# Samirez/Visual_odometry

Measured on AMD Instinct MI355X. Metric: frame-pairs/sec (1280x720, 2000 ORB feats), higher is better.
Workload: dtype u8+f32+f64; 1 GPU; seeded synthetic 1280x720 drone flight (256 distinct rendered views, closed loop), 2000 ORB features/frame, 8 levels = BASELINE config 2; chunk of 257 consecutive frames -> 256 pairs (k, k+1) per GPU per step, each frame detected once; detector=orb, distinct_rendered_frames=256, pair_stride=1, contexts_per_gpu=3, keypoint_order=cv2, poly_solver=fast, matcher=crosscheck, matcher_kernel=mfma_fp4, ransac=5-point, conf 0.99, 1 px, seed 2^64-1, <=1000 iters, parallelism=single GPU, pairs_ok_last_step=256

## Files before the change

### visual_odometry_amd/csrc/orb_kernels.hip

```cpp
#include "vo_internal.h"
#include <type_traits>
#include <float.h>
#include <stdlib.h>

__constant__ int8_t c_pattern[256 * 4] = {
#include "orb_pattern.inc"
};
__constant__ int c_umax[16] = {15, 15, 15, 15, 14, 14, 14, 13, 13, 12, 11, 10, 9, 8, 6, 3};
__constant__ int c_gauss7[7] = {18, 34, 49, 55, 49, 34, 18};


typedef short vo_s16x2 __attribute__((ext_vector_type(2)));
typedef unsigned short vo_u16x2 __attribute__((ext_vector_type(2)));
__device__ __forceinline__ uint32_t pk_sub16(uint32_t a, uint32_t b)
{
    return __builtin_bit_cast(uint32_t, __builtin_bit_cast(vo_s16x2, a) - __builtin_bit_cast(vo_s16x2, b));
}
__device__ __forceinline__ uint32_t pk_add16(uint32_t a, uint32_t b)
{
    return __builtin_bit_cast(uint32_t, __builtin_bit_cast(vo_s16x2, a) + __builtin_bit_cast(vo_s16x2, b));
}
__device__ __forceinline__ uint32_t pk_min16(uint32_t a, uint32_t b)
{
    return __builtin_bit_cast(uint32_t, __builtin_elementwise_min(__builtin_bit_cast(vo_s16x2, a), __builtin_bit_cast(vo_s16x2, b)));
// ... 1310 lines not shown
        uint32_t h0[4], h1[4];
        uint32_t a0 = src[0][0], a1 = src[0][1], a2 = src[0][2], b0 = src[1][0], b1 = src[1][1], b2 = src[1][2];
        if (EDGE) { bd_fix(a0, a1, a2, e); bd_fix(b0, b1, b2, e); }
        bd_hpass(a0, a1, a2, h0); bd_hpass(b0, b1, b2, h1);
#pragma unroll
        for (int c = 0; c < 4; c++) q[c] = h0[c] | (h1[c] << 16);
    };
#pragma unroll
    for (int u = 0; u < BD_AHEAD; u++) fetch(u, W[u]);
#pragma unroll
    for (int k = 0; k < 3; k++) {
        hstep(W[k % BD_AHEAD], Q[k % 4]);
        fetch(k + BD_AHEAD, W[k % BD_AHEAD]);
    }
    uint32_t orow = (uint32_t)(y0 * lv.stride);
    for (int m0 = 0; m0 < nsteps; m0 += 4) {
#pragma unroll
        for (int j = 0; j < 4; j++) {
            const int m = m0 + j;
            if (m >= nsteps) break;
            constexpr int K0 = 3;
            const int ki = (K0 + j) % 4, wi = (K0 + j) % BD_AHEAD;
            hstep(W[wi], Q[ki]);
            fetch(K0 + m + BD_AHEAD, W[wi]);
            const uint32_t r0 = bd_vrow<false>(Q[(ki + 1) % 4], Q[(ki + 2) % 4], Q[(ki + 3) % 4], Q[ki]);
            const uint32_t r1 = bd_vrow<true>(Q[(ki + 1) % 4], Q[(ki + 2) % 4], Q[(ki + 3) % 4], Q[ki]);
            __builtin_amdgcn_raw_buffer_store_b32(r0, drs, col_ok ? (uint32_t)x + orow : 0xfffffff0u, 0, 0);
            __builtin_amdgcn_raw_buffer_store_b32(r1, drs, col_ok && 2 * m + 1 < nout ? (uint32_t)x + orow + (uint32_t)lv.stride : 0xfffffff0u, 0, 0);
            orow += 2u * (uint32_t)lv.stride;
        }
    }
}

__global__ __launch_bounds__(256) void k_blur_direct(const uint8_t* pyr, uint8_t* blur, PyrGeom g, int total)
{
    const int f = blockIdx.y, lane = threadIdx.x & 63, wave = __builtin_amdgcn_readfirstlane(threadIdx.x >> 6);
    const int wt = xcd_tile(blockIdx.x, gridDim.x) * 4 + wave;
    if (wt >= total) return;
    int l = 0, first = 0;
    for (;;) {
        const int nt = ((g.lv[l].stride + 255) / 256) * ((g.lv[l].h + BD_R - 1) / BD_R);
        if (wt < first + nt || l + 1 == g.nlevels) break;
        first += nt; l++;
    }
    const LevelGeom lv = g.lv[l];
    const int ntx = (lv.stride + 255) / 256, tile = wt - first;
    const int x0 = (tile % ntx) * 256, y0 = (tile / ntx) * BD_R;
    const int x = x0 + 4 * lane;
    const uint8_t* img = pyr + (size_t)f * g.frame_bytes + lv.off;
    const int xb = min(max(x - 4, 0), lv.stride - 12);
    BdEdge e;
    e.left = x0 == 0; e.right = x0 + 256 + 8 > lv.w;
    e.shl = x == 0; e.shr = x - 4 > lv.stride - 12 && x < lv.stride;
    {
        const int d = lv.w - x;
        e.s1 = d == 1 ? 0x01020304u : d == 2 ? 0x03040504u : d == 3 ? 0x05060504u : 0x07060504u;
        e.s2 = d == 2 ? 0x0c0c0c02u : d == 3 ? 0x0c0c0304u : 0x0c040506u;
        e.s3 = d == 5 ? 0x01020304u : d == 6 ? 0x03040504u : 0x07060504u;
        e.use_t = d >= 2 && d <= 4;
    }
    const __amdgpu_buffer_rsrc_t drs = __builtin_amdgcn_make_buffer_rsrc(blur + (size_t)f * g.frame_bytes + lv.off, 0, lv.stride * lv.h, 0x00020000);
    const bool col_ok = x < lv.stride;
    const int nout = min(BD_R, lv.h - y0);
    const int nsteps = (nout + 1) / 2;
    const bool inside = y0 >= 3 && y0 - 3 + 2 * (nsteps + 3 + BD_AHEAD) <= lv.h, edge = e.left || e.right;
    if (inside && !edge) bd_strip<true, false>(img, lv, drs, x, xb, y0, nout, nsteps, col_ok, e);
    else if (inside) bd_strip<true, true>(img, lv, drs, x, xb, y0, nout, nsteps, col_ok, e);
    else if (!edge) bd_strip<false, false>(img, lv, drs, x, xb, y0, nout, nsteps, col_ok, e);
    else bd_strip<false, true>(img, lv, drs, x, xb, y0, nout, nsteps, col_ok, e);
}

void launch_blur(hipStream_t s, const uint8_t* pyr, uint8_t* blur, const PyrGeom& g, int F)
{
    bool direct = true;
    int total = 0;
    for (int l = 0; l < g.nlevels; l++) {
        direct = direct && g.lv[l].w >= 16 && g.lv[l].h >= 8;
        total += ((g.lv[l].stride + 255) / 256) * ((g.lv[l].h + BD_R - 1) / BD_R);
    }
    if (direct) { hipLaunchKernelGGL(k_blur_direct, dim3((total + 3) / 4, F), dim3(256), 0, s, pyr, blur, g, total); return; }
    hipLaunchKernelGGL(k_blur, dim3(g.btiles_total, F), dim3(256), 0, s, pyr, blur, g);
}

__device__ __forceinline__ uint32_t brief_expand4(uint32_t nib)
{
    const uint32_t m = (nib * 0x00204081u) & 0x01010101u;
    return 0x81818181u ^ (m * 0xfeu);
}

__device__ __forceinline__ uint32_t brief_expand8_fp4(uint32_t b)
{
    uint32_t w = (b | (b << 12)) & 0x000F000Fu;
    w = (w | (w << 6)) & 0x03030303u;
    w = (w | (w << 3)) & 0x11111111u;
    return 0xAAAAAAAAu ^ (w << 3);
}

__global__ __launch_bounds__(256) void k_brief_trig(PyrGeom g, FrameFeat ff)
{
    const int f = blockIdx.y, k = blockIdx.x * 256 + threadIdx.x;
    if (k >= min(ff.kp_count[f], g.kp_cap)) return;
    const size_t ki = (size_t)f * g.kp_cap + k;
    const float angle = ff.kp_angle[ki] * (float)(3.1415926535897932384626433832795 / 180.f);
    ff.kp_xy[ki * 2] = (float)cos((double)angle);
    ff.kp_xy[ki * 2 + 1] = (float)sin((double)angle);
}

#define BR_R 18
#define BR_ROWS (2 * BR_R + 1)
#ifndef BR_KPW
#define BR_KPW 2
#endif
__global__ __launch_bounds__(256) void k_brief(const uint8_t* blur, PyrGeom g, FrameFeat ff, uint8_t* desc_x, int cap_x, int blocks_per_frame, int fp4)
{
    __shared__ __attribute__((aligned(16))) uint8_t s_win[4][BR_KPW][BR_ROWS * 64];
    const int bid = xcd_tile(blockIdx.x, gridDim.x);
    const int f = bid / blocks_per_frame, lane = threadIdx.x & 63, wave = threadIdx.x >> 6;
    const int k0 = ((bid % blocks_per_frame) * 4 + wave) * BR_KPW;
    const int cnt = min(ff.kp_count[f], g.kp_cap);
    if (k0 >= cnt) return;
    float ca[BR_KPW], cb[BR_KPW], kxs[BR_KPW], kys[BR_KPW], sfs[BR_KPW];
    int coff[BR_KPW];
    uint4 wv[BR_KPW][3];
#pragma unroll
    for (int q = 0; q < BR_KPW; q++) {
        const size_t ki = (size_t)f * g.kp_cap + min(k0 + q, cnt - 1);
        const uint32_t pos = __builtin_amdgcn_readfirstlane(ff.kp_pos[ki]);
        const int level = __builtin_amdgcn_readfirstlane(ff.kp_level[ki]);
        const float sf = g.lv[level].scale;
        const int stride = g.lv[level].stride, lh = g.lv[level].h;
        const float kx = (float)(pos & 0xffff) * sf, ky = (float)(pos >> 16) * sf;
        const float inv = 1.f / sf;
        const int cx = __float2int_rn(kx * inv), cy = __float2int_rn(ky * inv);
        ca[q] = ff.kp_xy[ki * 2]; cb[q] = ff.kp_xy[ki * 2 + 1];
        kxs[q] = kx; kys[q] = ky; sfs[q] = sf;
        const uint8_t* img = blur + (size_t)f * g.frame_bytes + g.lv[level].off;
        const int xs = (cx - BR_R) & ~15;
        const int nchunk = (cx - BR_R - xs) + 2 * BR_R + 1 > 48 ? 4 : 3;
        coff[q] = BR_R * 64 + (cx - xs);
#pragma unroll
        for (int it = 0; it < 3; it++) {
            const int idx = min(it * 64 + lane, BR_ROWS * 4 - 1);
            const int r = idx >> 2, c = idx & 3;
            const int gy = min(max(cy - BR_R + r, 0), lh - 1), gx = min(max(xs + (c < nchunk ? 16 * c : 0), 0), stride - 16);
            wv[q][it] = *(const uint4*)(img + (size_t)gy * stride + gx);
        }
    }
#pragma unroll
    for (int q = 0; q < BR_KPW; q++)
#pragma unroll
        for (int it = 0; it < 3; it++) {
            const int idx = it * 64 + lane;
            if (idx < BR_ROWS * 4) *(uint4*)(s_win[wave][q] + idx * 16) = wv[q][it];
        }
#pragma unroll
    for (int q = 0; q < BR_KPW; q++) {
        const int k = k0 + q;
        if (k >= cnt) break;
        const size_t ki = (size_t)f * g.kp_cap + k;
        const uint8_t* center = s_win[wave][q] + coff[q];
        const float a = ca[q], b = cb[q];
        uint64_t words[4];
#pragma unroll
        for (int w = 0; w < 4; w++) {
            const int8_t* pt = c_pattern + (w * 64 + lane) * 4;
            const float px0 = (float)pt[0], py0 = (float)pt[1], px1 = (float)pt[2], py1 = (float)pt[3];
            const float xa = px0 * a - py0 * b, ya = px0 * b + py0 * a;
            const float xb = px1 * a - py1 * b, yb = px1 * b + py1 * a;
            const int t0 = center[__float2int_rn(ya) * 64 + __float2int_rn(xa)];
            const int t1 = center[__float2int_rn(yb) * 64 + __float2int_rn(xb)];
            words[w] = __ballot(t0 < t1);
        }
        if (lane < 4) {
            uint64_t wv8 = lane == 0 ? words[0] : lane == 1 ? words[1] : lane == 2 ? words[2] : words[3];
            *(uint64_t*)(ff.desc + ki * 32 + lane * 8) = wv8;
        }
        if (fp4 < 0) {
        } else if (fp4) {
            if (lane < 8) {
                const uint64_t wv8 = lane < 2 ? words[0] : lane < 4 ? words[1] : lane < 6 ? words[2] : words[3];
                const uint32_t bits = (uint32_t)(wv8 >> (32 * (lane & 1)));
                const uint4 o = make_uint4(brief_expand8_fp4(bits & 255u), brief_expand8_fp4((bits >> 8) & 255u), brief_expand8_fp4((bits >> 16) & 255u), brief_expand8_fp4(bits >> 24));
                *(uint4*)(desc_x + ((size_t)f * cap_x * 16 + (size_t)(k & ~15) * 8 + (size_t)lane * 16 + (k & 15)) * 16) = o;
            }
        } else if (lane < 16) {
            const uint64_t wv8 = lane < 4 ? words[0] : lane < 8 ? words[1] : lane < 12 ? words[2] : words[3];
            const uint32_t bits = (uint32_t)(wv8 >> (16 * (lane & 3))) & 0xffffu;
            const uint4 o = make_uint4(brief_expand4(bits & 15u), brief_expand4((bits >> 4) & 15u), brief_expand4((bits >> 8) & 15u), brief_expand4(bits >> 12));
            *(uint4*)(desc_x + (((size_t)f * cap_x + (k & ~15)) * 16 + (size_t)lane * 16 + (k & 15)) * 16) = o;
        }
        if (lane == 0) {
            ff.kp_xy[ki * 2] = kxs[q]; ff.kp_xy[ki * 2 + 1] = kys[q];
            ff.kp_size[ki] = 31 * sfs[q];
        }
    }
}

void launch_brief(hipStream_t s, const uint8_t* blur, const PyrGeom& g, FrameFeat ff, int F, uint8_t* desc_x, int cap_x, int fp4)
{
    hipLaunchKernelGGL(k_brief_trig, dim3((g.kp_cap + 255) / 256, F), dim3(256), 0, s, g, ff);
    const int bpf = (g.kp_cap + 4 * BR_KPW - 1) / (4 * BR_KPW);
    hipLaunchKernelGGL(k_brief, dim3(bpf * F), dim3(256), 0, s, blur, g, ff, desc_x, cap_x, bpf, -1);
    launch_desc_expand(s, ff.desc, ff.kp_count, g.kp_cap, cap_x, desc_x, F, fp4);
}
```

### visual_odometry_amd/csrc/vo_api.hip

```cpp
#include "vo_internal.h"
#include <float.h>
#include <math.h>
#include <stdio.h>
#include <stdlib.h>
#include <string.h>
#include <vector>
#include <type_traits>
#include <algorithm>

#define MAX_EVENTS 384

struct DevList {
    struct Entry { void* p; bool pinned; };
    std::vector<Entry> ptrs;
    DevList() = default;
    DevList(const DevList&) = delete;
    DevList& operator=(DevList&& o) noexcept { if (this != &o) { release(); ptrs.swap(o.ptrs); } return *this; }
    ~DevList() { release(); }
    template <typename T> hipError_t alloc(T** p, size_t n) { return keep(hipMalloc((void**)p, (n ? n : 1) * sizeof(T)), (void**)p, false); }
    template <typename T> hipError_t alloc_pinned(T** p, size_t n)
    {
        return keep(hipHostMalloc((void**)p, (n ? n : 1) * sizeof(T), hipHostMallocDefault), (void**)p, true);
    }
    void release()
// ... 407 lines not shown
}

extern "C" int vo_set_poly_solver(vo_ctx* ctx, int kind)
{
    if (!ctx) return VO_ERR_INVALID;
    if (kind != 0 && kind != 1) FAIL(VO_ERR_INVALID, "poly solver must be 0 (noise-floor exit) or 1 (OpenCV's fixed 300 sweeps)");
    ctx->dk_early = kind == 0;
    return VO_OK;
}

extern "C" int vo_set_pnp_refine(vo_ctx* ctx, int kind)
{
    if (!ctx) return VO_ERR_INVALID;
    if (kind != 0 && kind != 1) FAIL(VO_ERR_INVALID, "pnp refine must be 1 (cv2's solvePnP(ITERATIVE) on the inliers) or 0 (fast minimiser from the RANSAC model)");
    ctx->pnp_refine = kind;
    return VO_OK;
}

extern "C" const char* vo_last_error(const vo_ctx* ctx) { return ctx ? ctx->err : "ctx is NULL"; }

extern "C" int vo_batch_configure(vo_ctx* ctx, int h, int w, const vo_orb_params* params, int max_frames, int max_pairs)
{
    if (!ctx) return VO_ERR_INVALID;
    int rc = check_params(ctx, params);
    if (rc) return rc;
    if (h < 1 || w < 1 || max_frames < 1 || max_pairs < 1) FAIL(VO_ERR_INVALID, "bad sizes");
    HIPCHK(hipSetDevice(ctx->device));
    if (ctx->configured && ctx->h == h && ctx->w == w && memcmp(&ctx->params, params, sizeof(*params)) == 0 &&
        ctx->max_frames >= max_frames && ctx->max_pairs >= max_pairs && ctx->pb_cap == ctx->g.kp_cap) {
        ctx->detector = 0;
        clear_last_run(ctx);
        return VO_OK;
    }
    HIPCHK(hipStreamSynchronize(ctx->stream));
    free_config(ctx);
    PyrGeom g;
    rc = make_geometry(ctx, h, w, params, &g);
    if (rc) return rc;
    ctx->g = g; ctx->h = h; ctx->w = w; ctx->params = *params;
    ctx->max_frames = max_frames; ctx->max_pairs = max_pairs;

    size_t tab_ints = 0, tab_u16 = 0;
    for (int l = 1; l < g.nlevels; l++) { tab_ints += g.lv[l].w + g.lv[l].h; tab_u16 += g.lv[l].w + g.lv[l].h; }
    std::vector<int> hofs(tab_ints + 1);
    std::vector<uint16_t> hc(tab_u16 + 1);
    const size_t int_bytes = (tab_ints + 1) * sizeof(int);
    DevList& m = ctx->orb_mem;
    uint8_t* tab_mem = nullptr;
    HIPCHK(m.alloc(&tab_mem, int_bytes + (tab_u16 + 1) * sizeof(uint16_t) + 64));
    int* d_ofs = (int*)tab_mem;
    uint16_t* d_c = (uint16_t*)(tab_mem + int_bytes);
    size_t oi = 0;
    for (int l = 1; l < g.nlevels; l++) {
        ResizeTab& t = ctx->tabs[l];
        const LevelGeom &s = g.lv[l - 1], &d = g.lv[l];
        build_lin_tab(s.w, d.w, &hofs[oi], &hc[oi], &t.min_x, &t.max_x);
        t.xofs = d_ofs + oi; t.xc1 = d_c + oi; oi += d.w;
        build_lin_tab(s.h, d.h, &hofs[oi], &hc[oi], &t.min_y, &t.max_y);
        t.yofs = d_ofs + oi; t.yc1 = d_c + oi; oi += d.h;
        {
            const int* xo = &hofs[oi - d.h - d.w]; const int* yo = &hofs[oi - d.h];
            bool ok = true;
            for (int x = 0; x + 3 < d.w && ok; x++) ok = xo[x + 3] - xo[x] <= 4;
            for (int y = 0; y + 1 < d.h && ok; y++) ok = yo[y + 1] > yo[y];
            for (int y0 = 0; y0 < d.h && ok; y0 += RS2_WH) { const int yl = (y0 + RS2_WH < d.h ? y0 + RS2_WH : d.h) - 1; ok = yo[yl] + 2 - yo[y0] <= (RS2_WH * 127 + 99) / 100 + 3; }
            t.direct = ok ? 1 : 0;
        }
    }
    HIPCHK(hipMemcpy(d_ofs, hofs.data(), int_bytes, hipMemcpyHostToDevice));
    HIPCHK(hipMemcpy(d_c, hc.data(), (tab_u16 + 1) * sizeof(uint16_t), hipMemcpyHostToDevice));

    const size_t F = (size_t)max_frames, fb = (size_t)g.frame_bytes;
    HIPCHK(m.alloc(&ctx->pyr, F * fb + 256));
    HIPCHK(m.alloc(&ctx->blur, F * fb));
    HIPCHK(m.alloc(&ctx->score, F * fb));
    HIPCHK(hipMemset(ctx->pyr, 0, F * fb));
    FrameFeat& ff = ctx->ff;
    HIPCHK(m.alloc(&ff.cand_pos, F * g.cand_total)); HIPCHK(m.alloc(&ff.cand_resp, F * g.cand_total));
    HIPCHK(m.alloc(&ff.cand_count, F * VO_MAX_LEVELS));
    HIPCHK(m.alloc(&ff.kp_pos, F * g.kp_cap)); HIPCHK(m.alloc(&ff.kp_level, F * g.kp_cap));
    HIPCHK(m.alloc(&ff.kp_resp, F * g.kp_cap)); HIPCHK(m.alloc(&ff.kp_angle, F * g.kp_cap));
    HIPCHK(m.alloc(&ff.kp_xy, F * g.kp_cap * 2)); HIPCHK(m.alloc(&ff.kp_size, F * g.kp_cap));
    HIPCHK(m.alloc(&ff.desc, F * g.kp_cap * 32));
    HIPCHK(m.alloc(&ctx->desc_x, F * (size_t)desc_x_rows(g.kp_cap) * 256));
    HIPCHK(hipMemset(ctx->desc_x, 0xFF, F * (size_t)desc_x_rows(g.kp_cap) * 256));
    HIPCHK(m.alloc(&ff.kp_count, F)); HIPCHK(m.alloc(&ff.flags, F));
    HIPCHK(m.alloc(&ff.hist, F * VO_MAX_LEVELS * 256));
    HIPCHK(m.alloc(&ff.tile_list, F * (size_t)g.ftiles_total * FAST_LISTCAP));
    HIPCHK(m.alloc(&ff.tile_count, F * (size_t)g.ftiles_total));
    HIPCHK(m.alloc(&ctx->sel_thr, F * VO_MAX_LEVELS));
    HIPCHK(m.alloc(&ctx->har_kept, F * VO_MAX_LEVELS));
    HIPCHK(m.alloc(&ctx->har_thr, F * VO_MAX_LEVELS));
    HIPCHK(m.alloc(&ctx->sel_chunk_count, F * (size_t)(g.sel_chunks_total + 1)));
    HIPCHK(hipMemset(ff.kp_count, 0, F * sizeof(int)));
    HIPCHK(hipMemset(ff.flags, 0, F * sizeof(int)));
    HIPCHK(alloc_pairbuf(ctx->pb_mem, ctx->pb, max_pairs, g.kp_cap, false));
    ctx->pb_pairs = max_pairs; ctx->pb_cap = g.kp_cap;
    HIPCHK(hipDeviceSynchronize());
    ctx->configured = true;
    ctx->detector = 0;
    if (ctx->kp_order == 1) { rc = alloc_cv2(ctx); if (rc) return rc; }
    return VO_OK;
}

struct Batch {
    bool sift, ready;
    int w, h, max_frames, max_pairs, kp_cap;
    const uint8_t *desc, *desc_x; const float* kp_xy; const int *kp_count, *flags, *norms;
    int fp4;
    uint8_t* gray; int gray_stride; size_t gray_frame;
    uint8_t* gray_slot(int k) const { return gray + (size_t)k * gray_frame; }
};

static Batch batch(const vo_ctx* ctx)
{
    if (ctx->detector == 1) {
        const SiftState& S = ctx->sift;
        return {true, S.configured, S.w, S.h, S.max_frames, ctx->sift_pairs, S.kp_cap, S.desc, S.desc_x, S.kp_xy, S.kp_count, S.flags, S.norms, 0,
                S.frames, S.fstride, (size_t)S.fstride * S.h};
    }
    const PyrGeom& g = ctx->g;
    return {false, ctx->configured, ctx->w, ctx->h, ctx->max_frames, ctx->max_pairs, g.kp_cap, ctx->ff.desc, ctx->desc_x, ctx->ff.kp_xy,
            ctx->ff.kp_count, ctx->ff.flags, nullptr, ctx->descx_fp4, ctx->pyr + g.lv[0].off, g.lv[0].stride, (size_t)g.frame_bytes};
}

static void gray_into_slots(vo_ctx* ctx, hipStream_t s, const uint8_t* src, int channels, int row_stride, int64_t frame_stride, int first_slot, int n)
{
    const Batch b = batch(ctx);
    if (b.sift) launch_gray_plain(s, src, channels, row_stride, frame_stride, b.gray_slot(first_slot), b.w, b.h, b.gray_stride, (int64_t)b.gray_frame, n);
    else launch_gray(s, src, channels, row_stride, frame_stride, ctx->pyr + (size_t)first_slot * ctx->g.frame_bytes, ctx->g, n);
}

static int frames_upload_enqueue(vo_ctx* ctx, const uint8_t* frames, int F, int row_stride, int64_t frame_stride, int first_slot)
{
    const Batch b = batch(ctx);
    if (!b.ready) FAIL(VO_ERR_NOT_CONFIGURED, "vo_batch_configure has not been called");
    if (!frames || F < 0 || first_slot < 0 || first_slot + F > b.max_frames) FAIL(VO_ERR_INVALID, "slot range out of bounds");
    if (row_stride < b.w) FAIL(VO_ERR_INVALID, "row_stride < width");
    if (F == 0) return VO_OK;
    HIPCHK(hipSetDevice(ctx->device));
    if (b.sift) return sift_frames_upload_enqueue(ctx, frames, F, row_stride, frame_stride, first_slot);
    const LevelGeom& lv = ctx->g.lv[0];
    uint8_t* dst0 = ctx->pyr + (size_t)first_slot * ctx->g.frame_bytes + lv.off;
    if (row_stride == ctx->w && lv.stride == ctx->w && frame_stride >= (int64_t)ctx->w * ctx->h) {
        HIPCHK(hipMemcpy2DAsync(dst0, ctx->g.frame_bytes, frames, (size_t)frame_stride, (size_t)ctx->w * ctx->h, F,
                                hipMemcpyHostToDevice, ctx->stream));
        return VO_OK;
    }
    if (row_stride == ctx->w && frame_stride >= (int64_t)ctx->w * ctx->h) {
        const size_t per = (size_t)ctx->w * ctx->h;
        int rc = ctx->staging.grow(ctx, per * F); if (rc) return rc;
        HIPCHK(hipMemcpy2DAsync(ctx->staging.p, per, frames, (size_t)frame_stride, per, F, hipMemcpyHostToDevice, ctx->stream));
        launch_gray(ctx->stream, ctx->staging.p, 1, ctx->w, (int64_t)per, ctx->pyr + (size_t)first_slot * ctx->g.frame_bytes, ctx->g, F);
        HIPCHK(hipGetLastError());
        return VO_OK;
    }
    for (int f = 0; f < F; f++)
        HIPCHK(hipMemcpy2DAsync(dst0 + (size_t)f * ctx->g.frame_bytes, lv.stride, frames + (size_t)f * frame_stride, row_stride,
                                ctx->w, ctx->h, hipMemcpyHostToDevice, ctx->stream));
    return VO_OK;
}

extern "C" int vo_frames_upload(vo_ctx* ctx, const uint8_t* frames, int F, int row_stride, int64_t frame_stride, int first_slot)
{
    if (!ctx) return VO_ERR_INVALID;
    int rc = frames_upload_enqueue(ctx, frames, F, row_stride, frame_stride, first_slot);
    if (rc) return rc;
    HIPCHK(hipStreamSynchronize(ctx->stream));
    return VO_OK;
}

extern "C" int vo_frames_upload_async(vo_ctx* ctx, const uint8_t* frames, int F, int row_stride, int64_t frame_stride, int first_slot)
{
    if (!ctx) return VO_ERR_INVALID;
    return frames_upload_enqueue(ctx, frames, F, row_stride, frame_stride, first_slot);
}

extern "C" int vo_frames_upload_color(vo_ctx* ctx, const uint8_t* frames, int F, int channels, int row_stride,
                                      int64_t frame_stride, int first_slot)
{
    if (!ctx) return VO_ERR_INVALID;
    if (channels == 1) return vo_frames_upload(ctx, frames, F, row_stride, frame_stride, first_slot);
    const Batch b = batch(ctx);
    if (!b.ready) FAIL(VO_ERR_NOT_CONFIGURED, "vo_batch_configure has not been called");
    if (channels != 3 && channels != 4) FAIL(VO_ERR_INVALID, "channels must be 1, 3 or 4");
    if (!frames || F < 0 || first_slot < 0 || first_slot + F > b.max_frames) FAIL(VO_ERR_INVALID, "slot range out of bounds");
    if (row_stride < b.w * channels || frame_stride < (int64_t)row_stride * b.h) FAIL(VO_ERR_INVALID, "strides too small");
    if (F == 0) return VO_OK;
    HIPCHK(hipSetDevice(ctx->device));
    const size_t per = (size_t)frame_stride;
    const int chunk = F < 64 ? F : 64;
    int rc = ctx->staging.grow(ctx, per * chunk); if (rc) return rc;
    for (int f0 = 0; f0 < F; f0 += chunk) {
        const int n = F - f0 < chunk ? F - f0 : chunk;
        HIPCHK(hipMemcpyAsync(ctx->staging.p, frames + (size_t)f0 * per, per * n, hipMemcpyHostToDevice, ctx->stream));
        StageTimer t(ctx, ST_GRAY);
        gray_into_slots(ctx, ctx->stream, ctx->staging.p, channels, row_stride, frame_stride, first_slot + f0, n);
    }
    HIPCHK(hipGetLastError());
    HIPCHK(hipStreamSynchronize(ctx->stream));
    if (ctx->prof) prof_collect(ctx);
    return VO_OK;
}

static int run_detect(vo_ctx* ctx, int first_slot, int F, int upto)
{
    const PyrGeom& g = ctx->g;
    hipStream_t s = ctx->stream;
    uint8_t* pyr = ctx->pyr + (size_t)first_slot * g.frame_bytes;
    uint8_t* blur = ctx->blur + (size_t)first_slot * g.frame_bytes;
    uint8_t* score = ctx->score + (size_t)first_slot * g.frame_bytes;
    FrameFeat ff = ctx->ff;
    ff.cand_pos += (size_t)first_slot * g.cand_total; ff.cand_resp += (size_t)first_slot * g.cand_total;
    ff.cand_count += (size_t)first_slot * VO_MAX_LEVELS;
    ff.kp_pos += (size_t)first_slot * g.kp_cap; ff.kp_level += (size_t)first_slot * g.kp_cap;
    ff.kp_resp += (size_t)first_slot * g.kp_cap; ff.kp_angle += (size_t)first_slot * g.kp_cap;
    ff.kp_xy += (size_t)first_slot * g.kp_cap * 2; ff.kp_size += (size_t)first_slot * g.kp_cap;
    ff.desc += (size_t)first_slot * g.kp_cap * 32;
    ff.kp_count += first_slot; ff.flags += first_slot;
    ff.hist += (size_t)first_slot * VO_MAX_LEVELS * 256;
    ff.tile_list += (size_t)first_slot * g.ftiles_total * FAST_LISTCAP; ff.tile_count += (size_t)first_slot * g.ftiles_total;
    {
        StageTimer t(ctx, ST_RESIZE);
        for (int l = 1; l < g.nlevels; l++) launch_resize(s, pyr, g, l, ctx->tabs[l], F);
    }
    if (upto < 1) return VO_OK;
    const bool cv2 = ctx->kp_order == 1 && ctx->cv2_ready;
    Cv2Buf cb = ctx->cv2;
    if (cv2) {
        const size_t fo = (size_t)first_slot;
        cb.all_pos += fo * cb.all_total; cb.all_resp += fo * cb.all_total; cb.work += fo * cb.all_total;
        cb.lpos += fo * cb.all_total; cb.rpos += fo * cb.all_total;
        cb.all_count += fo * VO_MAX_LEVELS; cb.chunk_count += fo * g.sel_chunks_total;
    }
    {
        StageTimer t(ctx, ST_MISC);
        HIPCHK(hipMemsetAsync(ff.hist, 0, (size_t)F * VO_MAX_LEVELS * 256 * sizeof(uint32_t), s));
        if (upto < 2) {
            HIPCHK(hipMemsetAsync(ff.flags, 0, (size_t)F * sizeof(int), s));
            HIPCHK(hipMemsetAsync(ff.cand_count, 0, (size_t)F * VO_MAX_LEVELS * sizeof(int), s));
            if (cv2) HIPCHK(hipMemsetAsync(cb.all_count, 0, (size_t)F * VO_MAX_LEVELS * sizeof(int), s));
        }
    }
    { StageTimer t(ctx, ST_FAST); launch_fast(s, pyr, score, ff.hist, g, F, upto < 2 ? nullptr : ff.tile_list, ff.tile_count); }
    if (upto < 2) return VO_OK;
    { StageTimer t(ctx, ST_SELECT_FAST); launch_select_fast(s, g, ff, F, ctx->sel_thr + (size_t)first_slot * VO_MAX_LEVELS, ctx->sel_chunk_count + (size_t)first_slot * g.sel_chunks_total, ff.tile_list, ff.tile_count, cv2 ? &cb : nullptr); }
    if (g.score_type == 0) { StageTimer t(ctx, ST_HARRIS); launch_harris(s, pyr, g, ff, F); }
    { StageTimer t(ctx, ST_SELECT_HARRIS); launch_select_harris(s, g, ff, F, ctx->har_thr + (size_t)first_slot * VO_MAX_LEVELS, ctx->har_kept + (size_t)first_slot * VO_MAX_LEVELS); }
    if (cv2) {
        StageTimer t(ctx, ST_CV2_ORDER);
        launch_cv2_order(s, g, ff, cb, F, ctx->har_kept + (size_t)first_slot * VO_MAX_LEVELS);
    }
    { StageTimer t(ctx, ST_ANGLE); launch_angle(s, pyr, g, ff, F); }
    { StageTimer t(ctx, ST_BLUR); launch_blur(s, pyr, blur, g, F); }
    {
        StageTimer t(ctx, ST_BRIEF);
        const int cx = desc_x_rows(g.kp_cap);
        ctx->descx_fp4 = nn_kernel(ctx, g.kp_cap) == NN_FP4;
        launch_brief(s, blur, g, ff, F, ctx->desc_x + (size_t)first_slot * cx * 256, cx, ctx->descx_fp4);
    }
    return VO_OK;
}

extern "C" int vo_batch_kp_capacity(vo_ctx* ctx)
{
    if (!ctx) return 0;
    const Batch b = batch(ctx);
    return b.ready ? b.kp_cap : 0;
}

extern "C" int vo_host_alloc(size_t bytes, void** out)
{
    if (!out) return VO_ERR_INVALID;
    *out = nullptr;
    return hipHostMalloc(out, bytes ? bytes : 1, hipHostMallocDefault) == hipSuccess ? VO_OK : VO_ERR_HIP;
}

extern "C" void vo_host_free(void* p)
{
    if (p) (void)hipHostFree(p);
}

static int detect_enqueue(vo_ctx* ctx, int first_slot, int F)
{
    const Batch b = batch(ctx);
    if (!b.ready) FAIL(VO_ERR_NOT_CONFIGURED, "vo_batch_configure has not been called");
    if (F < 0 || first_slot < 0 || first_slot + F > b.max_frames) FAIL(VO_ERR_INVALID, "slot range out of bounds");
    HIPCHK(hipSetDevice(ctx->device));
    if (F == 0) return VO_OK;
    if (b.sift) return sift_frames_detect_enqueue(ctx, first_slot, F);
    int rc = run_detect(ctx, first_slot, F, 2);
    if (rc) return rc;
    HIPCHK(hipGetLastError());
    return VO_OK;
}

extern "C" int vo_frames_detect_async(vo_ctx* ctx, int first_slot, int F)
{
    if (!ctx) return VO_ERR_INVALID;
    int rc = detect_enqueue(ctx, first_slot, F);
    if (rc) return rc;
// ... 2289 lines not shown
```

### visual_odometry_amd/csrc/vo_internal.h

```cpp
#pragma once
#include <hip/hip_runtime.h>
#include <stdint.h>
#include "../../include/vo_hip.h"

enum {
    ST_GRAY = 0, ST_RESIZE, ST_FAST, ST_SELECT_FAST, ST_HARRIS, ST_SELECT_HARRIS, ST_ANGLE,
    ST_BLUR, ST_BRIEF, ST_MATCH_NN, ST_MATCH_SELECT, ST_RANSAC, ST_POSE, ST_TRIANGULATE,
    ST_MISC, ST_RESERVED, ST_SIFT_SCALE, ST_SIFT_EXTREMA, ST_SIFT_ORIENT, ST_SIFT_SORT, ST_SIFT_DESC, ST_CV2_ORDER, ST_GATHER, ST_RESERVED2,
    ST_SLAM_PREPARE, ST_SLAM_BA, ST_SLAM_FILTER, ST_SLAM_LIMIT
};

struct LevelGeom {
    int w, h, stride, off;
    int quota;
    float scale;
    int ftile_base, ftiles_x;
    int fox, foy;
    int dtile_base, dtiles_x;
    int btile_base, btiles_x;
    int cand_off, cand_cap;
    int sel_chunk_base;
};

struct PyrGeom {
    int nlevels, frame_bytes;
    int edge, fast_thr, score_type, nfeatures;
    int ftiles_total, btiles_total, dtiles_total;
    int cand_total, kp_cap;
    int sel_chunks_total;
    LevelGeom lv[VO_MAX_LEVELS];
};

#define RS2_WW 256
#define RS2_WH 16
#ifndef RS2_WAVES
#define RS2_WAVES 4
#endif
#define RS2_THREADS (64 * RS2_WAVES)
#define RS2_TH (RS2_WAVES * RS2_WH)

struct ResizeTab {
    const int* xofs; const uint16_t* xc1;
    const int* yofs; const uint16_t* yc1;
    int min_x, max_x, min_y, max_y;
    int direct;
};

#ifndef FAST_TW
#define FAST_TW 112
#endif
#ifndef FAST_TH
#define FAST_TH 20
#endif
#define BLUR_TW 128
#ifndef BLUR_TH
#define BLUR_TH 48
#endif
#define FAST_LISTCAP ((FAST_TW / 2) * (FAST_TH / 2))

struct FrameFeat {
    uint32_t* cand_pos;
    float*    cand_resp;
    int*      cand_count;
    uint32_t* kp_pos;
    int*      kp_level;
    float*    kp_resp;
    float*    kp_angle;
    float*    kp_xy;
    float*    kp_size;
    uint8_t*  desc;
    int*      kp_count;
    int*      flags;
    uint32_t* hist;
    uint32_t* tile_list;
    int*      tile_count;
};

struct Cv2Buf {
    uint32_t* all_pos;
    float*    all_resp;
    int*      all_count;
    int*      chunk_count;
    uint2*    work;
    uint32_t* lpos;
    uint32_t* rpos;
    int all_off[VO_MAX_LEVELS], all_cap[VO_MAX_LEVELS], all_total;
};

struct PoseState {
    int active;
    int ninl;
    int good[4];
    double R1[9], R2[9], t[3];
};

struct PairBuf {
    int*      slots;
    int*      nn_idx;
    int*      nn_dist;
    int*      nn_idx2;
    int*      nn_dist2;
    int*      nn_colkey;
    int*      m_q;
    int*      m_t;
    float*    m_d;
    int*      m_count;
    double*   px1;
    double*   px2;
    double*   xn1;
    double*   xn2;
    uint8_t*  mask;
    double*   models;
    PoseState* pose_state;
    double*   in1;
    double*   in2;
    double*   ipx1;
    double*   ipx2;
    vo_pair_result* res;
    double*   X;
    uint8_t*  pose_mask;
};

struct RansacParams {
    double prob, thresh_px;
    int max_iters;
    uint64_t seed;
    double K[9];
    double dist_thresh;
    int dk_early;
};

const char* rccl_load(void);
const char* rccl_unique_id(uint8_t* id128);
const char* rccl_comm_init(void** comm, const uint8_t* id128, int rank, int world);
void rccl_comm_destroy(void* comm);
const char* rccl_comm_count(void* comm, int* n);
const char* rccl_all_gather_f64(void* comm, const double* send, double* recv, size_t count, hipStream_t s);
void launch_pack_records(hipStream_t s, const vo_pair_result* res, int B, int valid, double* rec);

void launch_gray(hipStream_t s, const uint8_t* src, int channels, int row_stride, int64_t frame_stride,
                 uint8_t* pyr, const PyrGeom& g, int F);
void launch_gray_plain(hipStream_t s, const uint8_t* src, int channels, int row_stride, int64_t frame_stride,
                       uint8_t* dst, int w, int h, int dstride, int64_t dframe, int F);
void launch_resize(hipStream_t s, uint8_t* pyr, const PyrGeom& g, int level, const ResizeTab& tab, int F);
void launch_fast(hipStream_t s, const uint8_t* pyr, uint8_t* score, uint32_t* hist, const PyrGeom& g, int F,
                 uint32_t* tile_list, int* tile_count);
void launch_select_fast(hipStream_t s, const PyrGeom& g, FrameFeat ff, int F, int* thr, int* chunk_count,
                        const uint32_t* tile_list, const int* tile_count, const Cv2Buf* cb);
void launch_harris(hipStream_t s, const uint8_t* pyr, const PyrGeom& g, FrameFeat ff, int F);
void launch_cv2_order(hipStream_t s, const PyrGeom& g, FrameFeat ff, Cv2Buf cb, int F, const int* kept);
void launch_retain_raw(hipStream_t s, const float* resp, int n, int n_points, uint2* a, uint32_t* lpos, uint32_t* rpos,
                       int* order, int* n_out);
void launch_select_harris(hipStream_t s, const PyrGeom& g, FrameFeat ff, int F, float* thr, int* kept);
// ... 166 lines not shown
```

Before: 99470 frame-pairs/s.

## Precompute BRIEF window records and software-pipeline window fetches in k_brief

The trig kernel now also computes a 32-byte per-keypoint record (cos/sin, window offset, stride, chunk info) and writes kp_xy/kp_size, so k_brief can load each record with one scalar load. k_brief now handles 8 keypoints per wave in a loop that double-buffers the LDS window and prefetches the next keypoint's window and record while the current one is being sampled. The intent is to hide global load latency and cut per-keypoint address arithmetic. In exchange there is an extra record buffer and its write/read traffic. Row clamping at image borders is replaced by clamping the whole window offset, which can change the sampled pixels near edges.

Result: no change. 99420 frame-pairs/s (-0.0%).

```diff
diff --git a/visual_odometry_amd/csrc/orb_kernels.hip b/visual_odometry_amd/csrc/orb_kernels.hip
--- a/visual_odometry_amd/csrc/orb_kernels.hip
+++ b/visual_odometry_amd/csrc/orb_kernels.hip
@@ -1416,19 +1416,8 @@
     hipLaunchKernelGGL(k_blur, dim3(g.btiles_total, F), dim3(256), 0, s, pyr, blur, g);
 }
 
-__device__ __forceinline__ uint32_t brief_expand4(uint32_t nib)
-{
-    const uint32_t m = (nib * 0x00204081u) & 0x01010101u;
-    return 0x81818181u ^ (m * 0xfeu);
-}
-
-__device__ __forceinline__ uint32_t brief_expand8_fp4(uint32_t b)
-{
-    uint32_t w = (b | (b << 12)) & 0x000F000Fu;
-    w = (w | (w << 6)) & 0x03030303u;
-    w = (w | (w << 3)) & 0x11111111u;
-    return 0xAAAAAAAAu ^ (w << 3);
-}
+#define BR_R 18
+#define BR_ROWS (2 * BR_R + 1)
 
 __global__ __launch_bounds__(256) void k_brief_trig(PyrGeom g, FrameFeat ff)
 {
@@ -1436,97 +1425,91 @@
     if (k >= min(ff.kp_count[f], g.kp_cap)) return;
     const size_t ki = (size_t)f * g.kp_cap + k;
     const float angle = ff.kp_angle[ki] * (float)(3.1415926535897932384626433832795 / 180.f);
-    ff.kp_xy[ki * 2] = (float)cos((double)angle);
-    ff.kp_xy[ki * 2 + 1] = (float)sin((double)angle);
-}
-
-#define BR_R 18
-#define BR_ROWS (2 * BR_R + 1)
+    const uint32_t pos = ff.kp_pos[ki];
+    const int level = ff.kp_level[ki];
+    const float sf = g.lv[level].scale;
+    const int stride = g.lv[level].stride;
+    const float kx = (float)(pos & 0xffff) * sf, ky = (float)(pos >> 16) * sf;
+    const float inv = 1.f / sf;
+    const int cx = __float2int_rn(kx * inv), cy = __float2int_rn(ky * inv);
+    const int xs = (cx - BR_R) & ~15;
+    BriefRec r;
+    r.c = (float)cos((double)angle); r.s = (float)sin((double)angle);
+    r.off = (uint32_t)min(max(g.lv[level].off + (cy - BR_R) * stride + xs, 0), g.frame_bytes - (BR_ROWS - 1) * stride - 64);
+    r.stride = stride;
+    r.nchunk = (cx - BR_R - xs) + 2 * BR_R + 1 > 48 ? 4 : 3;
+    r.coff = BR_R * 64 + (cx - xs);
+    r.pad[0] = r.pad[1] = 0;
+    ff.brief_rec[ki] = r;
+    ff.kp_xy[ki * 2] = kx; ff.kp_xy[ki * 2 + 1] = ky;
+    ff.kp_size[ki] = 31 * sf;
+}
+
 #ifndef BR_KPW
-#define BR_KPW 2
+#define BR_KPW 8
 #endif
-__global__ __launch_bounds__(256) void k_brief(const uint8_t* blur, PyrGeom g, FrameFeat ff, uint8_t* desc_x, int cap_x, int blocks_per_frame, int fp4)
-{
-    __shared__ __attribute__((aligned(16))) uint8_t s_win[4][BR_KPW][BR_ROWS * 64];
+typedef uint32_t br_rec8 __attribute__((ext_vector_type(8)));
+__device__ __forceinline__ br_rec8 brief_rec_load(const BriefRec* rec, int i)
+{
+    return *(const __attribute__((address_space(4))) br_rec8*)(uintptr_t)(rec + i);
+}
+
+__device__ __forceinline__ void brief_fetch(const uint8_t* img, const br_rec8& r, int c16, bool c3, int r0, int r2, uint4& w0, uint4& w1, uint4& w2)
+{
+    const uint32_t base = r[2] + (uint32_t)(c3 && r[4] == 3 ? 0 : c16);
+    const int stride = (int)r[3];
+    w0 = *(const uint4*)(img + (base + (uint32_t)__mul24(r0, stride)));
+    w1 = *(const uint4*)(img + (base + (uint32_t)__mul24(r0 + 16, stride)));
+    w2 = *(const uint4*)(img + (base + (uint32_t)__mul24(r2, stride)));
+}
+
+__global__ __launch_bounds__(256) void k_brief(const uint8_t* blur, int frame_bytes, int kp_cap, FrameFeat ff, int blocks_per_frame)
+{
+    __shared__ __attribute__((aligned(16))) uint8_t s_win[4][2][BR_ROWS * 64];
     const int bid = xcd_tile(blockIdx.x, gridDim.x);
-    const int f = bid / blocks_per_frame, lane = threadIdx.x & 63, wave = threadIdx.x >> 6;
+    const int f = bid / blocks_per_frame, lane = threadIdx.x & 63, wave = __builtin_amdgcn_readfirstlane(threadIdx.x >> 6);
     const int k0 = ((bid % blocks_per_frame) * 4 + wave) * BR_KPW;
-    const int cnt = min(ff.kp_count[f], g.kp_cap);
+    const int cnt = min(ff.kp_count[f], kp_cap);
     if (k0 >= cnt) return;
-    float ca[BR_KPW], cb[BR_KPW], kxs[BR_KPW], kys[BR_KPW], sfs[BR_KPW];
-    int coff[BR_KPW];
-    uint4 wv[BR_KPW][3];
-#pragma unroll
-    for (int q = 0; q < BR_KPW; q++) {
-        const size_t ki = (size_t)f * g.kp_cap + min(k0 + q, cnt - 1);
-        const uint32_t pos = __builtin_amdgcn_readfirstlane(ff.kp_pos[ki]);
-        const int level = __builtin_amdgcn_readfirstlane(ff.kp_level[ki]);
-        const float sf = g.lv[level].scale;
-        const int stride = g.lv[level].stride, lh = g.lv[level].h;
-        const float kx = (float)(pos & 0xffff) * sf, ky = (float)(pos >> 16) * sf;
-        const float inv = 1.f / sf;
-        const int cx = __float2int_rn(kx * inv), cy = __float2int_rn(ky * inv);
-        ca[q] = ff.kp_xy[ki * 2]; cb[q] = ff.kp_xy[ki * 2 + 1];
-        kxs[q] = kx; kys[q] = ky; sfs[q] = sf;
-        const uint8_t* img = blur + (size_t)f * g.frame_bytes + g.lv[level].off;
-        const int xs = (cx - BR_R) & ~15;
-        const int nchunk = (cx - BR_R - xs) + 2 * BR_R + 1 > 48 ? 4 : 3;
-        coff[q] = BR_R * 64 + (cx - xs);
-#pragma unroll
-        for (int it = 0; it < 3; it++) {
-            const int idx = min(it * 64 + lane, BR_ROWS * 4 - 1);
-            const int r = idx >> 2, c = idx & 3;
-            const int gy = min(max(cy - BR_R + r, 0), lh - 1), gx = min(max(xs + (c < nchunk ? 16 * c : 0), 0), stride - 16);
-            wv[q][it] = *(const uint4*)(img + (size_t)gy * stride + gx);
-        }
-    }
-#pragma unroll
-    for (int q = 0; q < BR_KPW; q++)
-#pragma unroll
-        for (int it = 0; it < 3; it++) {
-            const int idx = it * 64 + lane;
-            if (idx < BR_ROWS * 4) *(uint4*)(s_win[wave][q] + idx * 16) = wv[q][it];
-        }
-#pragma unroll
-    for (int q = 0; q < BR_KPW; q++) {
-        const int k = k0 + q;
-        if (k >= cnt) break;
-        const size_t ki = (size_t)f * g.kp_cap + k;
-        const uint8_t* center = s_win[wave][q] + coff[q];
-        const float a = ca[q], b = cb[q];
-        uint64_t words[4];
+    const int n = min(BR_KPW, cnt - k0);
+    float px0[4], py0[4], px1[4], py1[4];
+#pragma unroll
+    for (int w = 0; w < 4; w++) {
+        const int8_t* pt = c_pattern + (w * 64 + lane) * 4;
+        px0[w] = (float)pt[0]; py0[w] = (float)pt[1]; px1[w] = (float)pt[2]; py1[w] = (float)pt[3];
+    }
+    const uint8_t* img = blur + (size_t)f * frame_bytes;
+    const BriefRec* rec = ff.brief_rec + (size_t)f * kp_cap + k0;
+    uint8_t* desc = ff.desc + ((size_t)f * kp_cap + k0) * 32;
+    const int c16 = 16 * (lane & 3), r0 = lane >> 2, r2 = min(32 + r0, BR_ROWS - 1);
+    const bool c3 = (lane & 3) == 3;
+    uint4 w0, w1, w2;
+    br_rec8 rn = brief_rec_load(rec, 0);
+    brief_fetch(img, rn, c16, c3, r0, r2, w0, w1, w2);
+    br_rec8 rnn = brief_rec_load(rec, min(1, n - 1));
+    for (int i = 0; i < n; i++) {
+        uint8_t* win = s_win[wave][i & 1];
+        const float a = __uint_as_float(rn[0]), b = __uint_as_float(rn[1]);
+        const uint8_t* center = win + (int)rn[5];
+        *(uint4*)(win + lane * 16) = w0;
+        *(uint4*)(win + 1024 + lane * 16) = w1;
+        if (lane < BR_ROWS * 4 - 128) *(uint4*)(win + 2048 + lane * 16) = w2;
+        rn = rnn;
+        brief_fetch(img, rn, c16, c3, r0, r2, w0, w1, w2);
+        rnn = brief_rec_load(rec, min(i + 2, n - 1));
+        uint32_t lo[4], hi[4];
 #pragma unroll
         for (int w = 0; w < 4; w++) {
-            const int8_t* pt = c_pattern + (w * 64 + lane) * 4;
-            const float px0 = (float)pt[0], py0 = (float)pt[1], px1 = (float)pt[2], py1 = (float)pt[3];
-            const float xa = px0 * a - py0 * b, ya = px0 * b + py0 * a;
-            const float xb = px1 * a - py1 * b, yb = px1 * b + py1 * a;
-            const int t0 = center[__float2int_rn(ya) * 64 + __float2int_rn(xa)];
-            const int t1 = center[__float2int_rn(yb) * 64 + __float2int_rn(xb)];
-            words[w] = __ballot(t0 < t1);
-        }
-        if (lane < 4) {
-            uint64_t wv8 = lane == 0 ? words[0] : lane == 1 ? words[1] : lane == 2 ? words[2] : words[3];
-            *(uint64_t*)(ff.desc + ki * 32 + lane * 8) = wv8;
-        }
-        if (fp4 < 0) {
-        } else if (fp4) {
-            if (lane < 8) {
-                const uint64_t wv8 = lane < 2 ? words[0] : lane < 4 ? words[1] : lane < 6 ? words[2] : words[3];
-                const uint32_t bits = (uint32_t)(wv8 >> (32 * (lane & 1)));
-                const uint4 o = make_uint4(brief_expand8_fp4(bits & 255u), brief_expand8_fp4((bits >> 8) & 255u), brief_expand8_fp4((bits >> 16) & 255u), brief_expand8_fp4(bits >> 24));
-                *(uint4*)(desc_x + ((size_t)f * cap_x * 16 + (size_t)(k & ~15) * 8 + (size_t)lane * 16 + (k & 15)) * 16) = o;
-            }
-        } else if (lane < 16) {
-            const uint64_t wv8 = lane < 4 ? words[0] : lane < 8 ? words[1] : lane < 12 ? words[2] : words[3];
-            const uint32_t bits = (uint32_t)(wv8 >> (16 * (lane & 3))) & 0xffffu;
-            const uint4 o = make_uint4(brief_expand4(bits & 15u), brief_expand4((bits >> 4) & 15u), brief_expand4((bits >> 8) & 15u), brief_expand4(bits >> 12));
-            *(uint4*)(desc_x + (((size_t)f * cap_x + (k & ~15)) * 16 + (size_t)lane * 16 + (k & 15)) * 16) = o;
-        }
-        if (lane == 0) {
-            ff.kp_xy[ki * 2] = kxs[q]; ff.kp_xy[ki * 2 + 1] = kys[q];
-            ff.kp_size[ki] = 31 * sfs[q];
-        }
+            const float xa = px0[w] * a - py0[w] * b, ya = px0[w] * b + py0[w] * a;
+            const float xb = px1[w] * a - py1[w] * b, yb = px1[w] * b + py1[w] * a;
+            const int t0 = center[(int)__builtin_fmaf(rintf(ya), 64.f, rintf(xa))];
+            const int t1 = center[(int)__builtin_fmaf(rintf(yb), 64.f, rintf(xb))];
+            const uint64_t word = __ballot(t0 < t1);
+            lo[w] = (uint32_t)word; hi[w] = (uint32_t)(word >> 32);
+        }
+        const bool odd = lane & 1, upper = lane & 2;
+        const uint2 o = make_uint2(upper ? (odd ? lo[3] : lo[2]) : (odd ? lo[1] : lo[0]), upper ? (odd ? hi[3] : hi[2]) : (odd ? hi[1] : hi[0]));
+        if (lane < 4) *(uint2*)(desc + i * 32 + lane * 8) = o;
     }
 }
 
@@ -1534,6 +1517,6 @@
 {
     hipLaunchKernelGGL(k_brief_trig, dim3((g.kp_cap + 255) / 256, F), dim3(256), 0, s, g, ff);
     const int bpf = (g.kp_cap + 4 * BR_KPW - 1) / (4 * BR_KPW);
-    hipLaunchKernelGGL(k_brief, dim3(bpf * F), dim3(256), 0, s, blur, g, ff, desc_x, cap_x, bpf, -1);
+    hipLaunchKernelGGL(k_brief, dim3(bpf * F), dim3(256), 0, s, blur, g.frame_bytes, g.kp_cap, ff, bpf);
     launch_desc_expand(s, ff.desc, ff.kp_count, g.kp_cap, cap_x, desc_x, F, fp4);
 }
diff --git a/visual_odometry_amd/csrc/vo_api.hip b/visual_odometry_amd/csrc/vo_api.hip
--- a/visual_odometry_amd/csrc/vo_api.hip
+++ b/visual_odometry_amd/csrc/vo_api.hip
@@ -513,6 +513,7 @@
     HIPCHK(m.alloc(&ff.kp_resp, F * g.kp_cap)); HIPCHK(m.alloc(&ff.kp_angle, F * g.kp_cap));
     HIPCHK(m.alloc(&ff.kp_xy, F * g.kp_cap * 2)); HIPCHK(m.alloc(&ff.kp_size, F * g.kp_cap));
     HIPCHK(m.alloc(&ff.desc, F * g.kp_cap * 32));
+    HIPCHK(m.alloc(&ff.brief_rec, F * g.kp_cap));
     HIPCHK(m.alloc(&ctx->desc_x, F * (size_t)desc_x_rows(g.kp_cap) * 256));
     HIPCHK(hipMemset(ctx->desc_x, 0xFF, F * (size_t)desc_x_rows(g.kp_cap) * 256));
     HIPCHK(m.alloc(&ff.kp_count, F)); HIPCHK(m.alloc(&ff.flags, F));
@@ -647,7 +648,7 @@
     ff.kp_pos += (size_t)first_slot * g.kp_cap; ff.kp_level += (size_t)first_slot * g.kp_cap;
     ff.kp_resp += (size_t)first_slot * g.kp_cap; ff.kp_angle += (size_t)first_slot * g.kp_cap;
     ff.kp_xy += (size_t)first_slot * g.kp_cap * 2; ff.kp_size += (size_t)first_slot * g.kp_cap;
-    ff.desc += (size_t)first_slot * g.kp_cap * 32;
+    ff.desc += (size_t)first_slot * g.kp_cap * 32; ff.brief_rec += (size_t)first_slot * g.kp_cap;
     ff.kp_count += first_slot; ff.flags += first_slot;
     ff.hist += (size_t)first_slot * VO_MAX_LEVELS * 256;
     ff.tile_list += (size_t)first_slot * g.ftiles_total * FAST_LISTCAP; ff.tile_count += (size_t)first_slot * g.ftiles_total;
diff --git a/visual_odometry_amd/csrc/vo_internal.h b/visual_odometry_amd/csrc/vo_internal.h
--- a/visual_odometry_amd/csrc/vo_internal.h
+++ b/visual_odometry_amd/csrc/vo_internal.h
@@ -58,6 +58,16 @@
 #endif
 #define FAST_LISTCAP ((FAST_TW / 2) * (FAST_TH / 2))
 
+struct BriefRec {
+    float c, s;
+    uint32_t off;
+    int stride;
+    int nchunk;
+    int coff;
+    int pad[2];
+};
+static_assert(sizeof(BriefRec) == 32, "k_brief loads a record as eight dwords");
+
 struct FrameFeat {
     uint32_t* cand_pos;
     float*    cand_resp;
@@ -69,6 +79,7 @@
     float*    kp_xy;
     float*    kp_size;
     uint8_t*  desc;
+    BriefRec* brief_rec;
     int*      kp_count;
     int*      flags;
     uint32_t* hist;
```
